# mickgordinier/DPX_GPU_Genomics_Project

Measured on AMD Instinct MI355X. Metric: GCUPS, higher is better.
Workload: dtype int16; 1 GPU; LSW 10000-pair 1024x1024 batch per GPU, int16 score matrix written to HBM; algorithm=LSW, pairs_per_gpu=10000, query_len=1024, reference_len=1024, match=3, mismatch=-1, gap=-2, parallelism=1 GPU, world_size=1, tune_placement=True, cells_per_gpu=10485760000, matrix_bytes_per_gpu=22261760000, precondition_fills=76, kernel=k_linear_fill_pk, rows_per_lane=16

## Files before the change

dpx_gpu_genomics_project_amd/csrc/dpx_kernels.hip:

```cpp
#include <hip/hip_runtime.h>
#include <stdint.h>

#include <type_traits>

#include "dpx_kernels.h"
#include "dpx_layout.h"
#include "dpx_prims.hpp"

namespace {

using dpx::pack_lo16;
using dpx::wave_shr1;
using dpx::wave_shl1;
using dpx::s16x2;
using dpx::u16x2;
using dpx::as_s16x2;
using dpx::as_u16x2;
using dpx::as_u32;

typedef unsigned int u32x4 __attribute__((ext_vector_type(4)));
typedef unsigned int u32x2 __attribute__((ext_vector_type(2)));

#ifndef DPX_NT_STORES
#define DPX_NT_STORES 0
// ... 538 lines not shown
    const unsigned char *rp = refs - skew;
    const unsigned nEff = nrows > 0 ? (unsigned)n : 0u;
    const int rpLast = n + skew;
    unsigned char *putPtr = tileL + lane * kStageLine;
    const unsigned char *fetchPtr[8];
#pragma unroll
    for (int k = 0; k < 8; k++) fetchPtr[k] = tileL + ((lane & ~7) | k) * kStageLine + (((lane + k) & 7) << 4);
    u32x4 pend[Q];
    int pendN = 0;
    int16_t *pendDst = nullptr;
    int bordG = (2 - skew) * gap;
    int rcN = rp[0];
    auto flush = [&]() __attribute__((always_inline)) {
#if DPX_EXP_QUAD == 1
        if (pendN == 77)
#endif
#pragma unroll
        for (int hq = 0; hq < Q; hq++)
            if (hq < pendN) stream_store(reinterpret_cast<u32x4 *>(pendDst + (hq << 9)), pend[hq]);
    };
    auto lane_step = [&](const int t, auto kTag) __attribute__((always_inline)) {
        constexpr int K = decltype(kTag)::value;
        const int tms = t - skew;
        const int rc = rcN;
        rcN = rp[min(t + 1, rpLast)];
        const int sh = wave_shr1(st.Hl[R - 1], 0);
        const int upinG = (l == 0) ? (LOCAL ? gap : bordG) : sh;
        if constexpr (!LOCAL) bordG += gap;
        if ((unsigned)tms < nEff) {
            int h[R];
            lin_cells_g<R, LOCAL>(st, upinG, rc, 0xFFFEu - (unsigned)tms, matchG, mismatchG, gap, h);
            if constexpr (STORE) {
#pragma unroll
                for (int hq = 0; hq < Q; hq++) {
                    u32x4 v = {pack_lo16(h[8 * hq + 0], h[8 * hq + 1]), pack_lo16(h[8 * hq + 2], h[8 * hq + 3]),
                               pack_lo16(h[8 * hq + 4], h[8 * hq + 5]), pack_lo16(h[8 * hq + 6], h[8 * hq + 7])};
#if DPX_EXP_QUAD != 2
                    *reinterpret_cast<u32x4 *>(putPtr + hq * 64 * kStageLine + (K << 4)) = v;
#else
                    pend[hq].y += v.x;
#endif
                }
            }
        }
        if constexpr (STORE) {
            flush();
            constexpr int O = (K + 1) & 7;
            const uint32_t r = rt[O];
            const bool valid = (uint32_t)t >= (r & 0xFFFFu) && (uint32_t)t <= (r >> 16);
            pendN = valid ? (int)nv[O] : 0;
#if DPX_EXP_QUAD == 3
            pendN = Q;
#endif
            pendDst = waveBase + (size_t)t * Stage::kStepElems + (lane << 3);
#pragma unroll
            for (int hq = 0; hq < Q; hq++)
#if DPX_EXP_QUAD == 2
                pend[hq].x += (uint32_t)t;
#else
                pend[hq] = *reinterpret_cast<const u32x4 *>(fetchPtr[O] + hq * 64 * kStageLine);
#endif
        }
    };
    {
        int t = 0;
        for (; t + 8 <= steps; t += 8) {
            lane_step(t + 0, std::integral_constant<int, 0>{}); lane_step(t + 1, std::integral_constant<int, 1>{});
            lane_step(t + 2, std::integral_constant<int, 2>{}); lane_step(t + 3, std::integral_constant<int, 3>{});
            lane_step(t + 4, std::integral_constant<int, 4>{}); lane_step(t + 5, std::integral_constant<int, 5>{});
            lane_step(t + 6, std::integral_constant<int, 6>{}); lane_step(t + 7, std::integral_constant<int, 7>{});
        }
        if (t + 0 < steps) lane_step(t + 0, std::integral_constant<int, 0>{});
        if (t + 1 < steps) lane_step(t + 1, std::integral_constant<int, 1>{});
        if (t + 2 < steps) lane_step(t + 2, std::integral_constant<int, 2>{});
        if (t + 3 < steps) lane_step(t + 3, std::integral_constant<int, 3>{});
        if (t + 4 < steps) lane_step(t + 4, std::integral_constant<int, 4>{});
        if (t + 5 < steps) lane_step(t + 5, std::integral_constant<int, 5>{});
        if (t + 6 < steps) lane_step(t + 6, std::integral_constant<int, 6>{});
    }
    if constexpr (STORE) flush();
    if constexpr (LOCAL) {
        int bestv = 0, bestrow = 0, bestcol = 0;
        lin_fold_keys<R, LOCAL>(st, row0, nrows, bestv, bestrow, bestcol);
        int *mine = reinterpret_cast<int *>(scratch + lane * 16);
        __builtin_amdgcn_fence(__ATOMIC_RELEASE, "wavefront");
        __builtin_amdgcn_wave_barrier();
        mine[0] = bestv; mine[1] = bestrow; mine[2] = bestcol;
        __builtin_amdgcn_fence(__ATOMIC_RELEASE, "wavefront");
        __builtin_amdgcn_wave_barrier();
        __builtin_amdgcn_fence(__ATOMIC_ACQUIRE, "wavefront");
        if (has && l == 0) {
            for (int k = 1; k < sl.num; k++) {
                const int *o = reinterpret_cast<const int *>(scratch + (lane + k) * 16);
                if (o[0] > bestv) { bestv = o[0]; bestrow = o[1]; bestcol = o[2]; }
            }
            a.score[p] = bestv; a.endRow[p] = bestv > 0 ? bestrow : 0; a.endCol[p] = bestv > 0 ? bestcol : 0;
        }
    } else {
        const int lm = (m - 1) / R, rm = (m - 1) % R;
        if (has && l == lm) {
            int v = st.Hl[0];
#pragma unroll
            for (int r = 1; r < R; r++) v = (r == rm) ? st.Hl[r] : v;
            a.score[p] = v - gap; a.endRow[p] = m; a.endCol[p] = n;
        }
    }
}

#define DPX_SPLIT_MAX_WAVES 16
template <int R, bool LOCAL>
__global__ void __launch_bounds__(64 * DPX_SPLIT_MAX_WAVES) k_linear_split(const dpx_fill_args a) {
    extern __shared__ __attribute__((aligned(16))) unsigned char smem[];
    constexpr int G = 8 / R;
    static_assert(R == 2 || R == 4 || R == 8, "rows per lane");
    const int lane = threadIdx.x & 63;
    const int w = __builtin_amdgcn_readfirstlane((int)(threadIdx.x >> 6));
    int p = blockIdx.x;
    if (a.order) p = a.order[p];
    const dpx_pair_dev pr = a.pairs[p];
    const int n = pr.n, m = pr.m;
    const int gap = a.gapOpen, matchG = a.match - gap, mismatchG = a.mismatch - gap;
    const int W = dpx_tiled_stripes(m, R);
    const unsigned char *ref = reinterpret_cast<const unsigned char *>(a.seq + pr.refIdx);
    const unsigned char *qry = reinterpret_cast<const unsigned char *>(a.seq + pr.qryIdx);
    int *ctrl = reinterpret_cast<int *>(smem);
    int *result = ctrl + 32;
    if (threadIdx.x < 32) ctrl[threadIdx.x] = 0;
    const unsigned char *refl = stage_bytes(smem + a.ldsRefOff + 64, ref, n, (int)threadIdx.x, (int)blockDim.x) - 64;
    __syncthreads();
    if (w >= W) return;
    int16_t *edgeMine = reinterpret_cast<int16_t *>(smem + a.ldsQryOff) + (size_t)w * a.ldsBufStride;
    const int16_t *edgePrev = edgeMine - a.ldsBufStride;

    const int row0 = w * 64 * R + lane * R;
    const int nrows = min(max(m - row0, 0), R);
    LinState<R, LOCAL> st;
    load_query_rows<R>(st.qc, qry, row0, nrows);
#pragma unroll
    for (int r = 0; r < R; r++) {
        st.Hl[r] = (LOCAL ? 0 : (row0 + 1 + r) * gap) + gap;
        st.key[r] = 0u;
    }
    st.dtop = (LOCAL ? 0 : row0 * gap) + gap;
    const bool hasNext = w + 1 < W;
    const int rowsHere = min(m - w * 64 * R, 64 * R);
    const int storeLanes = min(64, (((rowsHere + R - 1) / R) + 7) & ~7);
    const uint32_t SS = dpx_split_stripe_steps(n, R);
    const size_t cs = pr.chunkStride;
    int16_t *tile = a.mat + pr.matOff + ((size_t)w * (SS / G)) * cs + (size_t)lane * 8;
    const unsigned char *rp = refl + 64 - lane;
    auto wait_for = [&](const int need) {
        while (__hip_atomic_load(&ctrl[w - 1], __ATOMIC_ACQUIRE, __HIP_MEMORY_SCOPE_WORKGROUP) < need) __builtin_amdgcn_s_sleep(1);
    };
    int16_t *dump = reinterpret_cast<int16_t *>(smem + 384) + 16 * 0;
    uint32_t acc[4];
    int hv[R];
#pragma unroll
    for (int r = 0; r < R; r++) hv[r] = st.Hl[r] - gap;
    auto block16 = [&](const int tb, auto maskedTag) {
        constexpr bool MASKED = decltype(maskedTag)::value;
        if (w > 0) wait_for(min(tb + 17, n));
        int16_t *ew = (hasNext && lane == 63) ? edgeMine + (tb - 62) : dump;
        const unsigned char *rpb = rp + tb;
        const int16_t *epb = edgePrev + tb;
        int rcN = rpb[0];
        int e0N = ((w == 0) ? (LOCAL ? 0 : (tb + 1) * gap) : (int)epb[1]) + gap;
#pragma unroll
        for (int g = 0; g < 16; g++) {
            const int t = tb + g;
            const int rc = rcN, e0 = e0N;
            rcN = rpb[g + 1];
            e0N = ((w == 0) ? (LOCAL ? 0 : (t + 2) * gap) : (int)epb[g + 2]) + gap;
            const int upin = wave_shr1(st.Hl[R - 1], e0);
            const int j = t - lane + 1;
            const unsigned negj = 0xFFFFu - (unsigned)j;
            if constexpr (MASKED) {
                if (j >= 1 && j <= n) {
                    lin_cells_g<R, LOCAL>(st, upin, rc, negj, matchG, mismatchG, gap, hv);
                    if (hasNext && lane == 63) edgeMine[j] = (int16_t)hv[R - 1];
                }
            } else {
                lin_cells_g<R, LOCAL>(st, upin, rc, negj, matchG, mismatchG, gap, hv);
                ew[g] = (int16_t)hv[R - 1];
            }
            if constexpr (R == 8) {
                acc[0] = pack_lo16(hv[0], hv[1]); acc[1] = pack_lo16(hv[2], hv[3]);
                acc[2] = pack_lo16(hv[4], hv[5]); acc[3] = pack_lo16(hv[6], hv[7]);
            } else if constexpr (R == 4) {
                acc[2 * (g % G)] = pack_lo16(hv[0], hv[1]); acc[2 * (g % G) + 1] = pack_lo16(hv[2], hv[3]);
            } else {
                acc[g % G] = pack_lo16(hv[0], hv[1]);
            }
            if ((g % G) == G - 1 && t - (G - 1) < n + 63) {
                const bool doStore = lane < storeLanes;
                if (doStore) {
                    u32x4 v = {acc[0], acc[1], acc[2], acc[3]};
                    stream_store(reinterpret_cast<u32x4 *>(tile + (size_t)(t / G) * cs), v);
                }
            }
            if ((g & 7) == 7 && hasNext && t >= 63) {
                if (lane == 63) __hip_atomic_store(&ctrl[w], min(t - 62, n), __ATOMIC_RELEASE, __HIP_MEMORY_SCOPE_WORKGROUP);
            }
        }
    };
    {
        int tb = 0;
        const int steps = (int)SS;
        for (; tb < steps && tb < 64; tb += 16) block16(tb, std::true_type{});
        for (; tb + 16 <= n; tb += 16) block16(tb, std::false_type{});
        for (; tb < steps; tb += 16) block16(tb, std::true_type{});
    }
    if (hasNext && lane == 63) __hip_atomic_store(&ctrl[w], n, __ATOMIC_RELEASE, __HIP_MEMORY_SCOPE_WORKGROUP);

    int bestv = 0, bestrow = 0, bestcol = 0;
    if constexpr (LOCAL) {
        lin_fold_keys<R, LOCAL>(st, row0, nrows, bestv, bestrow, bestcol);
        const unsigned long long mine = ((unsigned long long)(unsigned)bestv << 32) | (unsigned)(0x7FFFFFFF - bestrow);
        const unsigned long long top = wave_max_u64(mine);
        if (mine == top && (bestv > 0 ? true : lane == 0)) { result[4 * w] = bestv; result[4 * w + 1] = bestrow; result[4 * w + 2] = bestcol; }
    } else {
        const int lm = (m - 1 - w * 64 * R) / R, rm = (m - 1) % R;
        if (w == W - 1 && lane == lm) {
            int v = st.Hl[0];
#pragma unroll
            for (int r = 1; r < R; r++) v = (r == rm) ? st.Hl[r] : v;
            a.score[p] = v - gap; a.endRow[p] = m; a.endCol[p] = n;
        }
    }
    if constexpr (LOCAL) {
        __builtin_amdgcn_fence(__ATOMIC_RELEASE, "workgroup");
        int arrived = 0;
        if (lane == 0) arrived = __hip_atomic_fetch_add(&ctrl[16], 1, __ATOMIC_ACQ_REL, __HIP_MEMORY_SCOPE_WORKGROUP);
        arrived = __builtin_amdgcn_readfirstlane(arrived);
        if (arrived == W - 1 && lane == 0) {
            int bv = 0, br = 0, bc = 0;
            for (int k = 0; k < W; k++) {
                const int v = __hip_atomic_load(&result[4 * k], __ATOMIC_RELAXED, __HIP_MEMORY_SCOPE_WORKGROUP);
                if (v > bv) { bv = v; br = result[4 * k + 1]; bc = result[4 * k + 2]; }
            }
            a.score[p] = bv; a.endRow[p] = bv > 0 ? br : 0; a.endCol[p] = bv > 0 ? bc : 0;
        }
    }
}

template <int R>
struct PkState {
    uint32_t Hl[R];
    uint32_t qc[R];
    uint32_t rmax[R];
    uint32_t rcol[R];
    uint32_t dtop;
    uint32_t keyA, keyB;
};

template <int R, int TAG>
__device__ __forceinline__ uint32_t pk_row_tag(uint32_t h) {
    static_assert(TAG >= 0 && TAG < R && R <= 16, "inline constants");
    uint32_t r;
    asm("v_pk_mad_u16 %0, %1, %2, %3 op_sel_hi:[1,0,0]" : "=v"(r) : "v"(h), "n"(R), "n"(TAG));
    return r;
}
template <int R>
__device__ __forceinline__ uint32_t pk_row_tag_of(uint32_t h, const int r) {
#define DPX_TAG_CASE(k) case k: if constexpr (k < R) return pk_row_tag<R, (k < R ? R - 1 - k : 0)>(h); else return 0u;
    switch (r) {
        DPX_TAG_CASE(0) DPX_TAG_CASE(1) DPX_TAG_CASE(2) DPX_TAG_CASE(3) DPX_TAG_CASE(4) DPX_TAG_CASE(5) DPX_TAG_CASE(6) DPX_TAG_CASE(7)
        DPX_TAG_CASE(8) DPX_TAG_CASE(9) DPX_TAG_CASE(10) DPX_TAG_CASE(11) DPX_TAG_CASE(12) DPX_TAG_CASE(13) DPX_TAG_CASE(14) DPX_TAG_CASE(15)
    default: return 0u;
    }
#undef DPX_TAG_CASE
}

__device__ __forceinline__ uint32_t pk_hi16(uint32_t lo, uint32_t hi) { return __builtin_amdgcn_perm(hi, lo, 0x07060302u); }

__device__ __forceinline__ s16x2 pk_gap_sat(const uint32_t up, const uint32_t left, const uint32_t gabsP) {
    return as_s16x2(as_u32(__builtin_elementwise_sub_sat(as_u16x2(as_u32(dpx::pk_max(as_s16x2(up), as_s16x2(left)))), as_u16x2(gabsP))));
}

template <int R>
__device__ __forceinline__ void store_tile_pk(int16_t *dstA, int16_t *dstB, const uint32_t (&v)[R]) {
    if constexpr (R == 2) {
        *reinterpret_cast<uint32_t *>(dstA) = pk_hi16(v[0], v[1]);
        *reinterpret_cast<uint32_t *>(dstB) = pack_lo16((int)v[0], (int)v[1]);
    } else if constexpr (R == 4) {
        uint2 a, b;
        a.x = pk_hi16(v[0], v[1]); a.y = pk_hi16(v[2], v[3]);
        b.x = pack_lo16((int)v[0], (int)v[1]); b.y = pack_lo16((int)v[2], (int)v[3]);
        *reinterpret_cast<uint2 *>(dstA) = a;
        *reinterpret_cast<uint2 *>(dstB) = b;
    } else {
#pragma unroll
        for (int q = 0; q < R / 8; q++) {
            uint4 a, b;
            a.x = pk_hi16(v[8 * q + 0], v[8 * q + 1]); a.y = pk_hi16(v[8 * q + 2], v[8 * q + 3]);
            a.z = pk_hi16(v[8 * q + 4], v[8 * q + 5]); a.w = pk_hi16(v[8 * q + 6], v[8 * q + 7]);
            b.x = pack_lo16((int)v[8 * q + 0], (int)v[8 * q + 1]); b.y = pack_lo16((int)v[8 * q + 2], (int)v[8 * q + 3]);
            b.z = pack_lo16((int)v[8 * q + 4], (int)v[8 * q + 5]); b.w = pack_lo16((int)v[8 * q + 6], (int)v[8 * q + 7]);
            *reinterpret_cast<uint4 *>(dstA + q * 512) = a;
            *reinterpret_cast<uint4 *>(dstB + q * 512) = b;
        }
    }
}

template <int R, bool LOCAL, bool MASKED, bool WHOLE, bool TAGS = false, bool PARTIAL = false>
__device__ __forceinline__ void pk_step(PkState<R> &st, const int t, const int lane, const int n, const bool laneHasRows, const int nrows,
                                        const uint32_t matchP, const uint32_t negDeltaP, const uint32_t gapP, const uint32_t e0,
                                        const uint32_t rcP, uint32_t *edge, const bool writeEdge, int16_t *tileA, int16_t *tileB,
                                        const int storeLanes, const int rampLines) {
    const int j = t - lane + 1;
    const uint32_t upin = (uint32_t)wave_shr1((int)st.Hl[R - 1], (int)e0);
    bool active = true;
    if constexpr (MASKED) active = laneHasRows && (j >= 1) && (j <= n);
    if (active) {
        uint32_t u = upin, d = st.dtop;
        const uint32_t onesP = 0x00010001u;
        const uint32_t negj = 0xFFFFu - (uint32_t)j;
        uint32_t colMax = 0u;
#pragma unroll
        for (int r = 0; r < R; r++) {
            const uint32_t left = st.Hl[r];
            const uint32_t differs = dpx::pk_min_u16_raw(st.qc[r] ^ rcP, onesP);
            const s16x2 sc = as_s16x2(dpx::pk_mad_i16_raw(differs, negDeltaP, matchP));
            s16x2 h;
            if constexpr (LOCAL && TAGS) {
                h = dpx::pk_max(pk_gap_sat(u, left, gapP), (s16x2)(as_s16x2(d) + sc));
            } else {
                const s16x2 g = dpx::pk_max(as_s16x2(u), as_s16x2(left)) + as_s16x2(gapP);
                h = dpx::pk_max(g, (s16x2)(as_s16x2(d) + sc));
                if constexpr (LOCAL) h = dpx::pk_max(h, as_s16x2(0u));
            }
            d = left;
            u = as_u32(h);
            st.Hl[r] = u;
            if constexpr (LOCAL && TAGS) {
                uint32_t tg = pk_row_tag_of<R>(u, r);
                if constexpr (PARTIAL) tg = (r < nrows) ? tg : 0u;
                colMax = r == 0 ? tg : dpx::pk_max_u16_raw(colMax, tg);
            } else if constexpr (LOCAL) {
                st.rmax[r] = max(st.rmax[r], (u & 0xFFFF0000u) | negj);
                st.rcol[r] = max(st.rcol[r], (u << 16) | negj);
            }
        }
        if constexpr (LOCAL && TAGS) {
            st.keyA = max(st.keyA, (colMax & 0xFFFF0000u) | negj);
            st.keyB = max(st.keyB, (colMax << 16) | negj);
        }
        st.dtop = upin;
        if (writeEdge && lane == 63) edge[j] = st.Hl[R - 1];
        if constexpr (MASKED && !WHOLE) store_tile_pk<R>(tileA, tileB, st.Hl);
    }
    if constexpr (!MASKED || WHOLE) {
        bool doStore = lane < storeLanes;
        if constexpr (MASKED) doStore = doStore && ramp_stores<R>(lane, t, n, rampLines);
        if (doStore) store_tile_pk<R>(tileA, tileB, st.Hl);
    }
}

#ifndef DPX_PK_MIN_BLOCKS
#define DPX_PK_MIN_BLOCKS 1
#endif
template <int R, bool LOCAL, bool TAGS>
__global__ void __launch_bounds__(DPX_FILL_THREADS, DPX_PK_MIN_BLOCKS) k_linear_fill_pk(const dpx_fill_args a) {
    extern __shared__ __attribute__((aligned(16))) unsigned char smem[];
    const int lane = threadIdx.x & 63;
    const int wv = __builtin_amdgcn_readfirstlane(threadIdx.x >> 6);
    const int c = blockIdx.x * (int)a.wavesPerBlock + wv;
    if (c >= a.numPairs) return;
    const int pA = a.order[2 * c], pB = a.order[2 * c + 1];
    const dpx_pair_dev prA = a.pairs[pA], prB = a.pairs[pB];
    const int n = prA.n, m = prA.m;
    const unsigned char *refA = reinterpret_cast<const unsigned char *>(a.seq + prA.refIdx);
    const unsigned char *refB = reinterpret_cast<const unsigned char *>(a.seq + prB.refIdx);
    const unsigned char *qryA = reinterpret_cast<const unsigned char *>(a.seq + prA.qryIdx);
    const unsigned char *qryB = reinterpret_cast<const unsigned char *>(a.seq + prB.qryIdx);
    const int gap = a.gapOpen;
    const uint32_t matchP = ((uint32_t)(uint16_t)a.match << 16) | (uint16_t)a.match;
    const uint32_t negDeltaP = ((uint32_t)(uint16_t)(a.mismatch - a.match) << 16) | (uint16_t)(a.mismatch - a.match);
    const int gapK = (LOCAL && TAGS) ? -gap : gap;
    const uint32_t gapP = ((uint32_t)(uint16_t)gapK << 16) | (uint16_t)gapK;

    unsigned char *my = smem + (size_t)wv * a.ldsPerWave;
    uint32_t *edge = reinterpret_cast<uint32_t *>(my);
    uint16_t *refl = reinterpret_cast<uint16_t *>(my + a.ldsRefOff);
    for (int x = 4 * lane; x < n; x += 256) {
        const uint32_t a4 = load4(refA + x), b4 = load4(refB + x);
        uint2 w;
        w.x = __builtin_amdgcn_perm(a4, b4, 0x05010400u);
        w.y = __builtin_amdgcn_perm(a4, b4, 0x07030602u);
        *reinterpret_cast<uint2 *>(refl + 64 + x) = w;
    }
    for (int x = lane; x <= n + 1; x += 64) {
        const uint16_t b = (uint16_t)(LOCAL ? 0 : x * gap);
        edge[x] = ((uint32_t)b << 16) | b;
    }
    int16_t *HpA = a.mat + prA.matOff, *HpB = a.mat + prB.matOff;
    const int W = n + 63;
    const int S = dpx_tiled_stripes(m, R);
    int bestA = 0, browA = 0, bcolA = 0, bestB = 0, browB = 0, bcolB = 0;
    PkState<R> st;

    for (int k = 0; k < S; k++) {
        const int base = k * 64 * R;
        const int row0 = base + lane * R;
        const int nrows = min(max(m - row0, 0), R);
        const bool laneHasRows = nrows > 0;
        const bool hasNext = (k + 1 < S);
        int qa[R], qb[R];
        load_query_rows<R>(qa, qryA, row0, nrows);
        load_query_rows<R>(qb, qryB, row0, nrows);
#pragma unroll
        for (int r = 0; r < R; r++) {
            st.qc[r] = ((uint32_t)qa[r] << 16) | (uint32_t)qb[r];
            const uint16_t b = (uint16_t)(LOCAL ? 0 : (row0 + 1 + r) * gap);
            st.Hl[r] = ((uint32_t)b << 16) | b;
            st.rmax[r] = 0u;
            st.rcol[r] = 0u;
        }
        st.keyA = st.keyB = 0u;
        { const uint16_t b = (uint16_t)(LOCAL ? 0 : row0 * gap); st.dtop = ((uint32_t)b << 16) | b; }
        const size_t csA = prA.chunkStride, csB = prB.chunkStride;
        int16_t *tileA = HpA + (size_t)k * (size_t)n * csA + (size_t)lane * (R < 8 ? R : 8);
        int16_t *tileB = HpB + (size_t)k * (size_t)n * csB + (size_t)lane * (R < 8 ? R : 8);
        const uint16_t *rp = refl + 64 - lane;
        uint32_t rcN = rp[0];
        uint32_t e0N = edge[1];
#define DPX_PK_STEP(MASKED_, WHOLE_, HASROWS_, PARTIAL_)                                                                        \
        {                                                                                                             \
            const uint32_t rc16 = rcN, e0 = e0N;                                                                      \
            rcN = rp[t + 1];                                                                                          \
            e0N = edge[min(t + 2, n + 1)];                                                                            \
            const uint32_t rcP = __builtin_amdgcn_perm(0u, rc16, 0x0c010c00u);   \
            pk_step<R, LOCAL, MASKED_, WHOLE_, TAGS, PARTIAL_>(st, t, lane, n, HASROWS_, nrows, matchP, negDeltaP, gapP, e0, rcP, edge, hasNext, \
                                       tileA + (size_t)t * csA, tileB + (size_t)t * csB, storeLanes, a.rampLines);   \
        }
        const bool fast = (base + 64 * R <= m) && (n >= 64);
        const int storeLanes = (S == 1) ? store_lanes<R>(m) : 64;
        if (S == 1) {
            if (fast) {
                int t = 0;
                for (; t < 63; t++) DPX_PK_STEP(true, true, true, false)
                for (; t + 1 < n;) { DPX_PK_STEP(false, true, true, false) t++; DPX_PK_STEP(false, true, true, false) t++; }
                for (; t < n; t++) DPX_PK_STEP(false, true, true, false)
                for (; t < W; t++) DPX_PK_STEP(true, true, true, false)
            } else {
                for (int t = 0; t < W; t++) DPX_PK_STEP(true, true, laneHasRows, true)
            }
        } else if (fast) {
            int t = 0;
            for (; t < 63; t++) DPX_PK_STEP(true, false, true, false)
            for (; t < n; t++) DPX_PK_STEP(false, false, true, false)
            for (; t < W; t++) DPX_PK_STEP(true, false, true, false)
        } else {
            for (int t = 0; t < W; t++) DPX_PK_STEP(true, false, laneHasRows, true)
        }
#undef DPX_PK_STEP
        if constexpr (LOCAL && TAGS) {
            constexpr int TB = R == 16 ? 4 : R == 8 ? 3 : R == 4 ? 2 : 1;
            const int hA = (int)(st.keyA >> (16 + TB)), hB = (int)(st.keyB >> (16 + TB));
            if (hA > bestA) { bestA = hA; browA = row0 + R - (int)((st.keyA >> 16) & (R - 1)); bcolA = 0xFFFF - (int)(st.keyA & 0xFFFFu); }
            if (hB > bestB) { bestB = hB; browB = row0 + R - (int)((st.keyB >> 16) & (R - 1)); bcolB = 0xFFFF - (int)(st.keyB & 0xFFFFu); }
        } else if constexpr (LOCAL) {
#pragma unroll
            for (int r = 0; r < R; r++) {
                const int hA = (int)(st.rmax[r] >> 16), hB = (int)(st.rcol[r] >> 16);
                if (r < nrows && hA > bestA) { bestA = hA; browA = row0 + 1 + r; bcolA = 0xFFFF - (int)(st.rmax[r] & 0xFFFFu); }
                if (r < nrows && hB > bestB) { bestB = hB; browB = row0 + 1 + r; bcolB = 0xFFFF - (int)(st.rcol[r] & 0xFFFFu); }
            }
        }
    }

    if constexpr (LOCAL) {
        const unsigned long long mineA = ((unsigned long long)(unsigned)bestA << 32) | (unsigned)(0x7FFFFFFF - browA);
        const unsigned long long mineB = ((unsigned long long)(unsigned)bestB << 32) | (unsigned)(0x7FFFFFFF - browB);
        const unsigned long long topA = wave_max_u64(mineA), topB = wave_max_u64(mineB);
        if ((int)(topA >> 32) == 0) { if (lane == 0) { a.score[pA] = 0; a.endRow[pA] = 0; a.endCol[pA] = 0; } }
        else if (mineA == topA) { a.score[pA] = bestA; a.endRow[pA] = browA; a.endCol[pA] = bcolA; }
        if ((int)(topB >> 32) == 0) { if (lane == 0) { a.score[pB] = 0; a.endRow[pB] = 0; a.endCol[pB] = 0; } }
        else if (mineB == topB) { a.score[pB] = bestB; a.endRow[pB] = browB; a.endCol[pB] = bcolB; }
    } else {
        const int lastBase = (S - 1) * 64 * R;
        const int lm = (m - 1 - lastBase) / R, rm = (m - 1 - lastBase) % R;
        if (lane == lm) {
            uint32_t v = st.Hl[0];
#pragma unroll
            for (int r = 1; r < R; r++) v = (r == rm) ? st.Hl[r] : v;
            a.score[pA] = (int)(int16_t)(v >> 16); a.endRow[pA] = m; a.endCol[pA] = n;
            a.score[pB] = (int)(int16_t)(v & 0xFFFFu); a.endRow[pB] = m; a.endCol[pB] = n;
        }
    }
}

template <bool LOCAL>
__global__ void __launch_bounds__(DPX_FILL_THREADS) k_linear_lanes_pk(const dpx_fill_args a) {
    extern __shared__ __attribute__((aligned(16))) unsigned char smem[];
    constexpr int kStageBytes = 2 * 64 * kStageLine;
    constexpr int kStepElems = 1024;
    const int lane = threadIdx.x & 63;
    const int wv = __builtin_amdgcn_readfirstlane(threadIdx.x >> 6);
    const int w = blockIdx.x * (int)a.wavesPerBlock + wv;
    if (w >= a.numPairs) return;
    const LaneSlot sl = find_slot(a.waves + w, lane);
    const bool has = sl.has;
    const int p = sl.p, l = sl.l;
    const dpx_pair_dev pr = a.pairs[p];
    const int n = has ? pr.n : 0, m = has ? pr.m : 0;
    const int gap = a.gapOpen;
    const uint32_t matchP = ((uint32_t)(uint16_t)a.match << 16) | (uint16_t)a.match;
    const uint32_t negDeltaP = ((uint32_t)(uint16_t)(a.mismatch - a.match) << 16) | (uint16_t)(a.mismatch - a.match);
    const int gapK = LOCAL ? -gap : gap;
    const uint32_t gapP = ((uint32_t)(uint16_t)gapK << 16) | (uint16_t)gapK;
    const unsigned char *ref = reinterpret_cast<const unsigned char *>(a.seq + pr.refIdx);
    const unsigned char *qry = reinterpret_cast<const unsigned char *>(a.seq + pr.qryIdx);

    unsigned char *tileL = smem + (size_t)wv * a.ldsPerWave;
    unsigned char *scratch = tileL;
    unsigned char *refl = tileL + kStageBytes + sl.refOff;
    const unsigned char *refs = stage_bytes(refl, ref, n, l, max(sl.num, 1));

    const int row0 = l * 16;
    const int nrows = min(max(m - row0, 0), 16);
    const int wmin = min(min(a.match, a.mismatch), min(gap, 0));
    const uint32_t negInf = (uint16_t)(-32768 - wmin);
    uint32_t Hl[8], qc[8], dtop, keyHi = 0u, keyLo = 0u;
    {
        int qa[16];
        load_query_rows<16>(qa, qry, row0, nrows);
#pragma unroll
        for (int r = 0; r < 8; r++) {
            qc[r] = ((uint32_t)qa[r] << 16) | (uint32_t)qa[8 + r];
            const uint16_t b = (uint16_t)(LOCAL ? 0 : (row0 + 1 + r) * gap);
            Hl[r] = ((uint32_t)b << 16) | negInf;
        }
        const uint16_t b = (uint16_t)(LOCAL ? 0 : row0 * gap);
        dtop = ((uint32_t)b << 16) | negInf;
    }
    const int first = lane - l;
    const int dOld = first & 7, dNew = (2 * first) & 7;
    const int skew = 2 * l + dNew;
    const int n8 = (n + 7) & ~7;
    const int LB = (int)dpx_tile8_row_blocks(m);
    const int nBlocks = has ? min(max(LB - 2 * l, 0), 2) : 0;
    {
        uint32_t *mine = reinterpret_cast<uint32_t *>(tileL + lane * kStageLine + 128);
        mine[0] = nBlocks >= 1 ? ((uint32_t)(skew + 7) | ((uint32_t)(n8 + skew - 1) << 16)) : 0x00007FFFu;
        mine[1] = nBlocks >= 2 ? ((uint32_t)(skew + 8) | ((uint32_t)(n8 + skew) << 16)) : 0x00007FFFu;
        mine[2] = (uint32_t)(skew - (l + dOld));
        __builtin_amdgcn_fence(__ATOMIC_RELEASE, "wavefront");
        __builtin_amdgcn_wave_barrier();
        __builtin_amdgcn_fence(__ATOMIC_ACQUIRE, "wavefront");
    }
    uint32_t rtHi[8], rtLo[8];
    int dl[8];
#pragma unroll
    for (int k = 0; k < 8; k++) {
        const uint32_t *o = reinterpret_cast<const uint32_t *>(tileL + ((lane & ~7) | k) * kStageLine + 128);
        rtHi[k] = o[0]; rtLo[k] = o[1]; dl[k] = (int)o[2];
    }
    int16_t *waveBase = a.mat + (size_t)(((unsigned long long)(unsigned)__builtin_amdgcn_readfirstlane((int)(pr.matOff >> 32)) << 32) |
                                         (unsigned)__builtin_amdgcn_readfirstlane((int)(pr.matOff & 0xFFFFFFFFull)));
    const int lastStep = has ? (nBlocks >= 2 ? n8 + skew : n8 + skew - 1) : -1;
    const int steps = __builtin_amdgcn_readfirstlane(wave_max_i32(lastStep)) + 1;
    const unsigned char *rp = refs - skew;
    const unsigned nEff = nrows > 8 ? (unsigned)n + 1u : (nrows > 0 ? (unsigned)n : 0u);
    const int rpLast = n + skew;
    unsigned char *putPtr = tileL + lane * kStageLine;
    const unsigned char *fetchPtr[8];
#pragma unroll
    for (int k = 0; k < 8; k++) fetchPtr[k] = tileL + ((lane & ~7) | k) * kStageLine + (((lane + 2 * k) & 7) << 4);
    const int laneElems = ((lane >> 3) << 6) + ((lane & 7) << 3);
    u32x4 pendA, pendB;
    bool okA = false, okB = false;
    int16_t *dstA = nullptr, *dstB = nullptr;
    uint32_t bord = (uint16_t)(-skew * gap);
    uint32_t rcCur = rp[0], rcPrev = 0u;
    auto flush = [&]() __attribute__((always_inline)) {
        if (okA) stream_store(reinterpret_cast<u32x4 *>(dstA), pendA);
        if (okB) stream_store(reinterpret_cast<u32x4 *>(dstB), pendB);
    };
    auto lane_step = [&](const int t, auto kTag) __attribute__((always_inline)) {
        constexpr int K = decltype(kTag)::value;
        const int tms = t - skew;
        const uint32_t rcP = (rcCur << 16) | rcPrev;
        rcPrev = rcCur;
        rcCur = rp[min(t + 1, rpLast)];
        const uint32_t sh = (uint32_t)wave_shr1((int)Hl[7], 0);
        uint32_t upin = __builtin_amdgcn_perm(sh, Hl[7], 0x05040302u);
        if constexpr (!LOCAL) bord = (uint32_t)(uint16_t)(bord + (uint32_t)gap);
        if (l == 0) upin = (LOCAL ? 0u : (bord << 16)) | (upin & 0xFFFFu);
        if ((unsigned)tms < nEff) {
            uint32_t u = upin, colMax = 0u;
            const uint32_t onesP = 0x00010001u;
            uint32_t dsum[8];
#pragma unroll
            for (int r = 0; r < 8; r++) {
                const uint32_t differs = dpx::pk_min_u16_raw(qc[r] ^ rcP, onesP);
                const uint32_t sc = dpx::pk_mad_i16_raw(differs, negDeltaP, matchP);
                dsum[r] = as_u32((s16x2)(as_s16x2(r == 0 ? dtop : Hl[r - 1]) + as_s16x2(sc)));
            }
#pragma unroll
            for (int r = 0; r < 8; r++) {
                s16x2 h;
                if constexpr (LOCAL) h = dpx::pk_max(pk_gap_sat(u, Hl[r], gapP), as_s16x2(dsum[r]));
                else h = dpx::pk_max(dpx::pk_max(as_s16x2(u), as_s16x2(Hl[r])) + as_s16x2(gapP), as_s16x2(dsum[r]));
                u = as_u32(h);
                Hl[r] = u;
                if constexpr (LOCAL) {
                    const uint32_t tg = pk_row_tag_of<8>(u, r);
                    colMax = r == 0 ? tg : dpx::pk_max_u16_raw(colMax, tg);
                }
            }
            dtop = upin;
            if constexpr (LOCAL) {
                const uint32_t negj = 0xFFFEu - (uint32_t)tms;
                if (tms < n) keyHi = max(keyHi, (colMax & 0xFFFF0000u) | negj);
                keyLo = max(keyLo, (colMax << 16) | (negj + 1u));
            }
            u32x4 vh = {pk_hi16(Hl[0], Hl[1]), pk_hi16(Hl[2], Hl[3]), pk_hi16(Hl[4], Hl[5]), pk_hi16(Hl[6], Hl[7])};
            u32x4 vl = {pack_lo16((int)Hl[0], (int)Hl[1]), pack_lo16((int)Hl[2], (int)Hl[3]), pack_lo16((int)Hl[4], (int)Hl[5]), pack_lo16((int)Hl[6], (int)Hl[7])};
            *reinterpret_cast<u32x4 *>(putPtr + (K << 4)) = vh;
            *reinterpret_cast<u32x4 *>(putPtr + 64 * kStageLine + (((K + 7) & 7) << 4)) = vl;
        }
        flush();
        constexpr int H = (K & 1) ? 0 : 1;
        constexpr int OA = (K & 1) ? (((K + 1) >> 1) & 3) : (K >> 1), OB = OA + 4;
        const uint32_t ra = H ? rtLo[OA] : rtHi[OA], rb = H ? rtLo[OB] : rtHi[OB];
        okA = (uint32_t)t >= (ra & 0xFFFFu) && (uint32_t)t <= (ra >> 16);
        okB = (uint32_t)t >= (rb & 0xFFFFu) && (uint32_t)t <= (rb >> 16);
        dstA = waveBase + (ptrdiff_t)(t - dl[OA] - H) * kStepElems + (H * 512 + laneElems);
        dstB = waveBase + (ptrdiff_t)(t - dl[OB] - H) * kStepElems + (H * 512 + laneElems);
        pendA = *reinterpret_cast<const u32x4 *>(fetchPtr[OA] + H * 64 * kStageLine);
        pendB = *reinterpret_cast<const u32x4 *>(fetchPtr[OB] + H * 64 * kStageLine);
    };
    {
        int t = 0;
        for (; t + 8 <= steps; t += 8) {
            lane_step(t + 0, std::integral_constant<int, 0>{}); lane_step(t + 1, std::integral_constant<int, 1>{});
            lane_step(t + 2, std::integral_constant<int, 2>{}); lane_step(t + 3, std::integral_constant<int, 3>{});
            lane_step(t + 4, std::integral_constant<int, 4>{}); lane_step(t + 5, std::integral_constant<int, 5>{});
            lane_step(t + 6, std::integral_constant<int, 6>{}); lane_step(t + 7, std::integral_constant<int, 7>{});
        }
        if (t + 0 < steps) lane_step(t + 0, std::integral_constant<int, 0>{});
        if (t + 1 < steps) lane_step(t + 1, std::integral_constant<int, 1>{});
        if (t + 2 < steps) lane_step(t + 2, std::integral_constant<int, 2>{});
        if (t + 3 < steps) lane_step(t + 3, std::integral_constant<int, 3>{});
        if (t + 4 < steps) lane_step(t + 4, std::integral_constant<int, 4>{});
        if (t + 5 < steps) lane_step(t + 5, std::integral_constant<int, 5>{});
        if (t + 6 < steps) lane_step(t + 6, std::integral_constant<int, 6>{});
    }
    flush();
    if constexpr (LOCAL) {
        int bestv = (int)(keyHi >> 19), bestrow = row0 + 8 - (int)((keyHi >> 16) & 7), bestcol = 0xFFFF - (int)(keyHi & 0xFFFFu);
        const int vLo = (int)(keyLo >> 19);
        if (vLo > bestv) { bestv = vLo; bestrow = row0 + 16 - (int)((keyLo >> 16) & 7); bestcol = 0xFFFF - (int)(keyLo & 0xFFFFu); }
        int *mine = reinterpret_cast<int *>(scratch + lane * 16);
        __builtin_amdgcn_fence(__ATOMIC_RELEASE, "wavefront");
        __builtin_amdgcn_wave_barrier();
        mine[0] = bestv; mine[1] = bestrow; mine[2] = bestcol;
        __builtin_amdgcn_fence(__ATOMIC_RELEASE, "wavefront");
        __builtin_amdgcn_wave_barrier();
        __builtin_amdgcn_fence(__ATOMIC_ACQUIRE, "wavefront");
        if (has && l == 0) {
            for (int k = 1; k < sl.num; k++) {
                const int *o = reinterpret_cast<const int *>(scratch + (lane + k) * 16);
                if (o[0] > bestv) { bestv = o[0]; bestrow = o[1]; bestcol = o[2]; }
            }
            a.score[p] = bestv; a.endRow[p] = bestv > 0 ? bestrow : 0; a.endCol[p] = bestv > 0 ? bestcol : 0;
        }
    } else {
        const int lm = (m - 1) / 16, rr = (m - 1) % 16;
        if (has && l == lm) {
            uint32_t v = Hl[0];
#pragma unroll
            for (int r = 1; r < 8; r++) v = (r == (rr & 7)) ? Hl[r] : v;
            a.score[p] = (rr < 8) ? (int)(int16_t)(v >> 16) : (int)(int16_t)(v & 0xFFFFu);
            a.endRow[p] = m; a.endCol[p] = n;
        }
    }
}

template <int R>
struct AffState {
    int Hl[R], Il[R];
    int Dl[R];
    int qc[R];
    unsigned key[R];
    int dtop;
};

template <int R, bool LOCAL>
__device__ __forceinline__ void aff_cells(AffState<R> &st, const int upH, const int upD, const int rc, const int match,
                                          const int mismatch, const int oe, const int e, const unsigned negj) {
    int uH = upH, uD = upD, d = st.dtop;
#pragma unroll
    for (int r = 0; r < R; r++) {
        const int lH = st.Hl[r];
        const int s = (st.qc[r] == rc) ? match : mismatch;
        const int Dn = max(uH + oe, uD + e);
        const int In = max(lH + oe, st.Il[r] + e);
        int h = max(max(Dn, d + s), In);
        if constexpr (LOCAL) {
            h = max(h, 0);
            st.key[r] = max(st.key[r], ((unsigned)h << 16) | negj);
        }
        d = lH;
        uH = h;
        uD = Dn;
        st.Hl[r] = h;
        st.Il[r] = In;
        st.Dl[r] = Dn;
    }
    st.dtop = upH;
}

template <int R, bool LOCAL, bool STORE, bool MASKED, bool WHOLE>
__device__ __forceinline__ void aff_step(AffState<R> &st, const int t, const int lane, const int n, const bool laneHasRows,
                                         const int match, const int mismatch, const int oe, const int e, const int e0H,
                                         const int e0D, const int rc, int16_t *edgeH, int16_t *edgeD,
                                         const bool writeEdge, int16_t *tileDst, const int storeLanes, const int rampLines) {
    const int j = t - lane + 1;
    const int upH = wave_shr1(st.Hl[R - 1], e0H);
    const int upD = wave_shr1(st.Dl[R - 1], e0D);
    bool active = true;
    if constexpr (MASKED) active = laneHasRows && (j >= 1) && (j <= n);
    if (active) {
        aff_cells<R, LOCAL>(st, upH, upD, rc, match, mismatch, oe, e, 0xFFFFu - (unsigned)j);
        if (writeEdge && lane == 63) {
            edgeH[j] = (int16_t)st.Hl[R - 1];
            edgeD[j] = (int16_t)st.Dl[R - 1];
        }
        if constexpr (STORE && MASKED && !WHOLE) {
            store_tile<R>(tileDst, st.Hl);
            store_tile<R>(tileDst + 64 * R, st.Il);
            store_tile<R>(tileDst + 128 * R, st.Dl);
        }
    }
    if constexpr (STORE && (!MASKED || WHOLE)) {
        bool doStore = lane < storeLanes;
        if constexpr (MASKED) doStore = doStore && ramp_stores<R>(lane, t, n, rampLines);
        if (doStore) {
            store_tile<R>(tileDst, st.Hl);
            store_tile<R>(tileDst + 64 * R, st.Il);
            store_tile<R>(tileDst + 128 * R, st.Dl);
        }
    }
}

template <int R>
__device__ __forceinline__ void fold_row_keys(const unsigned (&key)[R], const int row0, const int nrows, int &bestv, int &bestrow, int &bestcol) {
#pragma unroll
    for (int r = 0; r < R; r++) {
        const int hv = (int)(key[r] >> 16), col = 0xFFFF - (int)(key[r] & 0xFFFFu);
        if (r < nrows && hv > bestv) {
            bestv = hv;
            bestrow = row0 + 1 + r;
            bestcol = col;
        }
// ... 1483 lines not shown
```

Before: 3222 GCUPS.

## Software-pipeline packed LSW inner loop and drop edge traffic for single-stripe tiles

```diff
diff --git a/dpx_gpu_genomics_project_amd/csrc/dpx_kernels.hip b/dpx_gpu_genomics_project_amd/csrc/dpx_kernels.hip
--- a/dpx_gpu_genomics_project_amd/csrc/dpx_kernels.hip
+++ b/dpx_gpu_genomics_project_amd/csrc/dpx_kernels.hip
@@ -864,55 +864,128 @@
     }
 }
 
-template <int R, bool LOCAL, bool MASKED, bool WHOLE, bool TAGS = false, bool PARTIAL = false>
+__device__ __forceinline__ uint32_t pk_min1_u16(uint32_t x) {
+    uint32_t r;
+    asm("v_pk_min_u16 %0, %1, 1 op_sel_hi:[1,0]" : "=v"(r) : "v"(x));
+    return r;
+}
+__device__ __forceinline__ uint32_t pk_mad_i16_sk(uint32_t a, uint32_t k, uint32_t c) {
+    uint32_t r;
+    asm("v_pk_mad_i16 %0, %1, %2, %3" : "=v"(r) : "v"(a), "s"(k), "v"(c));
+    return r;
+}
+
+#define DPX_PK_PIN() __builtin_amdgcn_sched_barrier(0)
+#define DPX_PK_HOLD(v) asm volatile("" : "+v"(v))
+
+template <int R, bool LOCAL, bool MASKED, bool WHOLE, bool TAGS = false, bool PARTIAL = false, bool EDGE = true, bool FULL = false>
 __device__ __forceinline__ void pk_step(PkState<R> &st, const int t, const int lane, const int n, const bool laneHasRows, const int nrows,
                                         const uint32_t matchP, const uint32_t negDeltaP, const uint32_t gapP, const uint32_t e0,
                                         const uint32_t rcP, uint32_t *edge, const bool writeEdge, int16_t *tileA, int16_t *tileB,
                                         const int storeLanes, const int rampLines) {
+    constexpr bool PIPE = R == 16 && !(LOCAL && !TAGS);
     const int j = t - lane + 1;
-    const uint32_t upin = (uint32_t)wave_shr1((int)st.Hl[R - 1], (int)e0);
+    uint32_t upin;
+    if constexpr (!EDGE && LOCAL) upin = (uint32_t)__builtin_amdgcn_update_dpp(0, (int)st.Hl[R - 1], 0x138, 0xf, 0xf, true);
+    else upin = (uint32_t)wave_shr1((int)st.Hl[R - 1], (int)e0);
     bool active = true;
     if constexpr (MASKED) active = laneHasRows && (j >= 1) && (j <= n);
     if (active) {
-        uint32_t u = upin, d = st.dtop;
+        uint32_t u = upin;
         const uint32_t onesP = 0x00010001u;
+        uint32_t colMax = 0u;
         const uint32_t negj = 0xFFFFu - (uint32_t)j;
-        uint32_t colMax = 0u;
-#pragma unroll
-        for (int r = 0; r < R; r++) {
-            const uint32_t left = st.Hl[r];
-            const uint32_t differs = dpx::pk_min_u16_raw(st.qc[r] ^ rcP, onesP);
-            const s16x2 sc = as_s16x2(dpx::pk_mad_i16_raw(differs, negDeltaP, matchP));
-            s16x2 h;
-            if constexpr (LOCAL && TAGS) {
-                h = dpx::pk_max(pk_gap_sat(u, left, gapP), (s16x2)(as_s16x2(d) + sc));
-            } else {
-                const s16x2 g = dpx::pk_max(as_s16x2(u), as_s16x2(left)) + as_s16x2(gapP);
-                h = dpx::pk_max(g, (s16x2)(as_s16x2(d) + sc));
-                if constexpr (LOCAL) h = dpx::pk_max(h, as_s16x2(0u));
-            }
-            d = left;
-            u = as_u32(h);
-            st.Hl[r] = u;
-            if constexpr (LOCAL && TAGS) {
-                uint32_t tg = pk_row_tag_of<R>(u, r);
-                if constexpr (PARTIAL) tg = (r < nrows) ? tg : 0u;
-                colMax = r == 0 ? tg : dpx::pk_max_u16_raw(colMax, tg);
-            } else if constexpr (LOCAL) {
-                st.rmax[r] = max(st.rmax[r], (u & 0xFFFF0000u) | negj);
-                st.rcol[r] = max(st.rcol[r], (u << 16) | negj);
+        uint32_t tg = 0u;
+        if constexpr (!PIPE) {
+            uint32_t d = st.dtop;
+#pragma unroll
+            for (int r = 0; r < R; r++) {
+                const uint32_t left = st.Hl[r];
+                const uint32_t differs = dpx::pk_min_u16_raw(st.qc[r] ^ rcP, onesP);
+                const s16x2 sc = as_s16x2(dpx::pk_mad_i16_raw(differs, negDeltaP, matchP));
+                s16x2 h;
+                if constexpr (LOCAL && TAGS) {
+                    h = dpx::pk_max(pk_gap_sat(u, left, gapP), (s16x2)(as_s16x2(d) + sc));
+                } else {
+                    const s16x2 g = dpx::pk_max(as_s16x2(u), as_s16x2(left)) + as_s16x2(gapP);
+                    h = dpx::pk_max(g, (s16x2)(as_s16x2(d) + sc));
+                    if constexpr (LOCAL) h = dpx::pk_max(h, as_s16x2(0u));
+                }
+                d = left;
+                u = as_u32(h);
+                st.Hl[r] = u;
+                if constexpr (LOCAL && TAGS) {
+                    tg = pk_row_tag_of<R>(u, r);
+                    if constexpr (PARTIAL) tg = (r < nrows) ? tg : 0u;
+                    colMax = r == 0 ? tg : dpx::pk_max_u16_raw(colMax, tg);
+                } else if constexpr (LOCAL) {
+                    st.rmax[r] = max(st.rmax[r], (u & 0xFFFF0000u) | negj);
+                    st.rcol[r] = max(st.rcol[r], (u << 16) | negj);
+                }
+            }
+        } else {
+            uint32_t mn[R + 2], dsum[R + 1];
+    #pragma unroll
+            for (int r = 0; r < 2 && r < R; r++) mn[r] = pk_min1_u16(st.qc[r] ^ rcP);
+            dsum[0] = as_u32((s16x2)(as_s16x2(pk_mad_i16_sk(mn[0], negDeltaP, st.dtop)) + as_s16x2(matchP)));
+            DPX_PK_PIN();
+    #pragma unroll
+            for (int r = 0; r < R; r++) {
+                const uint32_t left = st.Hl[r];
+                const s16x2 m1 = dpx::pk_max(as_s16x2(u), as_s16x2(left));
+                DPX_PK_PIN();
+                uint32_t x = 0u, md = 0u;
+                if (r + 2 < R) {
+                    x = st.qc[r + 2] ^ rcP;
+                    if constexpr (LOCAL && TAGS) { if (r > 1) DPX_PK_HOLD(colMax); }
+                    DPX_PK_PIN();
+                }
+                if (r + 1 < R) { md = pk_mad_i16_sk(mn[r + 1], negDeltaP, left); DPX_PK_PIN(); }
+                s16x2 g;
+                if constexpr (LOCAL && TAGS)
+                    g = as_s16x2(as_u32(__builtin_elementwise_sub_sat(as_u16x2(as_u32(m1)), as_u16x2(gapP))));
+                else
+                    g = m1 + as_s16x2(gapP);
+                DPX_PK_PIN();
+                if (r + 1 < R) { dsum[r + 1] = as_u32((s16x2)(as_s16x2(md) + as_s16x2(matchP))); DPX_PK_PIN(); }
+                s16x2 h = dpx::pk_max(g, as_s16x2(dsum[r]));
+                DPX_PK_PIN();
+                if constexpr (LOCAL && TAGS) {
+                    if (r > 1) {
+                        if (r + 2 < R) colMax = as_u32(dpx::pk_max(as_u16x2(colMax), as_u16x2(tg)));
+                        else colMax = dpx::pk_max_u16_raw(colMax, tg);
+                        DPX_PK_PIN();
+                    } else if (r == 1) colMax = tg;
+                }
+                if (r + 2 < R) { mn[r + 2] = pk_min1_u16(x); DPX_PK_PIN(); }
+                u = as_u32(h);
+                st.Hl[r] = u;
+                if constexpr (LOCAL && TAGS) {
+                    if (r + 1 < R) {
+                        tg = pk_row_tag_of<R>(u, r);
+                        if constexpr (PARTIAL) tg = (r < nrows) ? tg : 0u;
+                        DPX_PK_PIN();
+                    }
+                }
             }
         }
         if constexpr (LOCAL && TAGS) {
+            if constexpr (PIPE) {
+                tg = pk_row_tag_of<R>(u, R - 1);
+                if constexpr (PARTIAL) tg = (R - 1 < nrows) ? tg : 0u;
+                colMax = as_u32(dpx::pk_max(as_u16x2(colMax), as_u16x2(tg)));
+            }
             st.keyA = max(st.keyA, (colMax & 0xFFFF0000u) | negj);
             st.keyB = max(st.keyB, (colMax << 16) | negj);
         }
         st.dtop = upin;
-        if (writeEdge && lane == 63) edge[j] = st.Hl[R - 1];
+        if constexpr (EDGE) { if (writeEdge && lane == 63) edge[j] = st.Hl[R - 1]; }
         if constexpr (MASKED && !WHOLE) store_tile_pk<R>(tileA, tileB, st.Hl);
     }
-    if constexpr (!MASKED || WHOLE) {
-        bool doStore = lane < storeLanes;
+    if constexpr (FULL && !MASKED) {
+        store_tile_pk<R>(tileA, tileB, st.Hl);
+    } else if constexpr (!MASKED || WHOLE) {
+        bool doStore = FULL ? true : (lane < storeLanes);
         if constexpr (MASKED) doStore = doStore && ramp_stores<R>(lane, t, n, rampLines);
         if (doStore) store_tile_pk<R>(tileA, tileB, st.Hl);
     }
@@ -951,13 +1024,16 @@
         w.y = __builtin_amdgcn_perm(a4, b4, 0x07030602u);
         *reinterpret_cast<uint2 *>(refl + 64 + x) = w;
     }
-    for (int x = lane; x <= n + 1; x += 64) {
-        const uint16_t b = (uint16_t)(LOCAL ? 0 : x * gap);
-        edge[x] = ((uint32_t)b << 16) | b;
+    const int S = dpx_tiled_stripes(m, R);
+    constexpr bool kLean = R == 16 && !(LOCAL && !TAGS);
+    if (S > 1 || !kLean) {
+        for (int x = lane; x <= n + 1; x += 64) {
+            const uint16_t b = (uint16_t)(LOCAL ? 0 : x * gap);
+            edge[x] = ((uint32_t)b << 16) | b;
+        }
     }
     int16_t *HpA = a.mat + prA.matOff, *HpB = a.mat + prB.matOff;
     const int W = n + 63;
-    const int S = dpx_tiled_stripes(m, R);
     int bestA = 0, browA = 0, bcolA = 0, bestB = 0, browB = 0, bcolB = 0;
     PkState<R> st;
 
@@ -985,14 +1061,15 @@
         int16_t *tileB = HpB + (size_t)k * (size_t)n * csB + (size_t)lane * (R < 8 ? R : 8);
         const uint16_t *rp = refl + 64 - lane;
         uint32_t rcN = rp[0];
-        uint32_t e0N = edge[1];
-#define DPX_PK_STEP(MASKED_, WHOLE_, HASROWS_, PARTIAL_)                                                                        \
+        uint32_t e0N = (S > 1 || !kLean) ? edge[1] : 0u;
+#define DPX_PK_STEP(MASKED_, WHOLE_, HASROWS_, PARTIAL_, EDGE_, FULL_)                                                          \
         {                                                                                                             \
-            const uint32_t rc16 = rcN, e0 = e0N;                                                                      \
+            const uint32_t rc16 = rcN;                                                                                \
+            const uint32_t e0 = EDGE_ ? e0N : (LOCAL ? 0u : (uint32_t)(uint16_t)((t + 1) * gap) * 0x00010001u);       \
             rcN = rp[t + 1];                                                                                          \
-            e0N = edge[min(t + 2, n + 1)];                                                                            \
+            if (EDGE_) e0N = edge[min(t + 2, n + 1)];                                                                 \
             const uint32_t rcP = __builtin_amdgcn_perm(0u, rc16, 0x0c010c00u);   \
-            pk_step<R, LOCAL, MASKED_, WHOLE_, TAGS, PARTIAL_>(st, t, lane, n, HASROWS_, nrows, matchP, negDeltaP, gapP, e0, rcP, edge, hasNext, \
+            pk_step<R, LOCAL, MASKED_, WHOLE_, TAGS, PARTIAL_, EDGE_, FULL_>(st, t, lane, n, HASROWS_, nrows, matchP, negDeltaP, gapP, e0, rcP, edge, hasNext, \
                                        tileA + (size_t)t * csA, tileB + (size_t)t * csB, storeLanes, a.rampLines);   \
         }
         const bool fast = (base + 64 * R <= m) && (n >= 64);
@@ -1000,20 +1077,20 @@
         if (S == 1) {
             if (fast) {
                 int t = 0;
-                for (; t < 63; t++) DPX_PK_STEP(true, true, true, false)
-                for (; t + 1 < n;) { DPX_PK_STEP(false, true, true, false) t++; DPX_PK_STEP(false, true, true, false) t++; }
-                for (; t < n; t++) DPX_PK_STEP(false, true, true, false)
-                for (; t < W; t++) DPX_PK_STEP(true, true, true, false)
+                for (; t < 63; t++) DPX_PK_STEP(true, true, true, false, !kLean, kLean)
+                for (; t + 1 < n;) { DPX_PK_STEP(false, true, true, false, !kLean, kLean) t++; DPX_PK_STEP(false, true, true, false, !kLean, kLean) t++; }
+                for (; t < n; t++) DPX_PK_STEP(false, true, true, false, !kLean, kLean)
+                for (; t < W; t++) DPX_PK_STEP(true, true, true, false, !kLean, kLean)
             } else {
-                for (int t = 0; t < W; t++) DPX_PK_STEP(true, true, laneHasRows, true)
+                for (int t = 0; t < W; t++) DPX_PK_STEP(true, true, laneHasRows, true, !kLean, false)
             }
         } else if (fast) {
             int t = 0;
-            for (; t < 63; t++) DPX_PK_STEP(true, false, true, false)
-            for (; t < n; t++) DPX_PK_STEP(false, false, true, false)
-            for (; t < W; t++) DPX_PK_STEP(true, false, true, false)
+            for (; t < 63; t++) DPX_PK_STEP(true, false, true, false, true, false)
+            for (; t < n; t++) DPX_PK_STEP(false, false, true, false, true, false)
+            for (; t < W; t++) DPX_PK_STEP(true, false, true, false, true, false)
         } else {
-            for (int t = 0; t < W; t++) DPX_PK_STEP(true, false, laneHasRows, true)
+            for (int t = 0; t < W; t++) DPX_PK_STEP(true, false, laneHasRows, true, true, false)
         }
 #undef DPX_PK_STEP
         if constexpr (LOCAL && TAGS) {
```

Result: no change. 3217 GCUPS (-0.1%).
